# xdsopl/dwt

Measured on AMD Instinct MI355X. Metric: Mpixels/s lossless encode+decode round-trip, higher is better.
Workload: dtype int32; 1 GPU; 4096x4096x1 8-bit synthetic smooth+noise frames, lossless, 128 frames per GPU per step (BASELINE.json configs[1] geometry); frames_per_gpu=128, parallelism=1 GPU

## Files before the change

### dwt_amd/csrc/dwtx_internal.h

```cpp
#pragma once

#include <hip/hip_runtime.h>
#include <stdint.h>
#include <stddef.h>
#include "../../include/dwtx.h"

#define DWTX_SCRATCH_SLOTS 24
#define DWTX_PART_STREAMS 4
#define DWTX_ENC_PARTS DWTX_PART_STREAMS

struct dwtx_linplan;

struct dwtx_ctx {
	int device;
	hipStream_t stream;
	bool own_stream;
	void *scratch[DWTX_SCRATCH_SLOTS];
	size_t scratch_bytes[DWTX_SCRATCH_SLOTS];
	dwtx_linplan *plans;
	hipStream_t side[DWTX_PART_STREAMS - 1];
	int nside;
	struct { hipEvent_t start, cleared, tables[DWTX_PART_STREAMS], scattered[DWTX_PART_STREAMS]; } dec_ev;
	dwtx_ctx *enc_part[DWTX_ENC_PARTS];
	struct { hipEvent_t start, lifted[DWTX_ENC_PARTS], done[DWTX_ENC_PARTS]; } enc_ev;
// ... 180 lines not shown
	p.kind = DWTX_SAMPLE_U16;
	return p;
}
static inline dwtx_pixels dwtx_pixels_float(void *pix, int kind, int channels, size_t image_stride, int maxval)
{
	dwtx_pixels p{ pix, kind == DWTX_SAMPLE_F32 ? 4 : 2, channels, image_stride, maxval };
	p.kind = kind;
	return p;
}

bool dwtx_pixels_ok(const dwtx_pixels &px, int W, int H);
int dwtx_lift_scratch(dwtx_ctx *ctx, int W, int H, int nplanes);
int dwtx_pixels_to_planes(dwtx_ctx *ctx, int32_t *planes, const dwtx_pixels &px, int W, int H, int n);
int dwtx_planes_to_pixels(dwtx_ctx *ctx, const dwtx_pixels &px, const int32_t *planes, int W, int H, int n);

struct dwtx_tiles {
	int NT;
	int tile_first[DWTX_MAX_LEVELS + 1];
	const int *base;
	const unsigned short *cnt;
	const int *blk;
	const int *xy2tile;
	int xy_first[DWTX_MAX_LEVELS + 1];
	int nbs[DWTX_MAX_LEVELS];
};

struct dwtx_hist_sink {
	unsigned *cum32;
	unsigned *tile_mx;
	int NT, NTP;
	dwtx_tiles tiles;
};
int dwtx_hist_begin(dwtx_ctx *ctx, int W, int H, int C, int n, dwtx_hist_sink *sink);
struct dwtx_p16 {
	int16_t *planes;
	unsigned levels;
};
int dwtx_fwd_pixels(dwtx_ctx *ctx, int32_t *out, const dwtx_pixels &px, int W, int H, int n, const dwtx_hist_sink *sink = nullptr,
	unsigned *hist_levels = nullptr, dwtx_p16 p16 = dwtx_p16{ nullptr, 0u });
int dwtx_inv_pixels(dwtx_ctx *ctx, const dwtx_pixels &px, const int32_t *in, int W, int H, int n, const dwtx_p16 *p16 = nullptr);
int dwtx_transformation_fwd_hist(dwtx_ctx *ctx, int32_t *out, const int32_t *in, int W, int H, int nplanes, const dwtx_hist_sink *sink,
	unsigned *hist_levels);
int dwtx_get_tiles(dwtx_ctx *ctx, int W, int H, dwtx_tiles *out);

template <class G> int dwtx_fill_geom(dwtx_ctx *ctx, int W, int H, int C, G &g, dwtx_tiles &tiles)
{
	int lengths[DWTX_MAX_LEVELS], pixels[DWTX_MAX_LEVELS], widths[DWTX_MAX_LEVELS], heights[DWTX_MAX_LEVELS];
	g.levels = dwtx_compute_lengths(lengths, pixels, widths, heights, W, H, DWTX_MIN_LEN);
	for (int l = 0; l <= g.levels; ++l) {
		g.pixels[l] = pixels[l];
		g.side[l] = l < g.levels ? lengths[l + 1] : 0;
	}
	g.C = C;
	g.W = W;
	g.H = H;
	g.total = (long)W * H;
	g.pyr = nullptr;
	g.fine16 = nullptr;
	g.lv16 = 0u;
	g.sq_levels = 0;
	const int rc = dwtx_get_tiles(ctx, W, H, &tiles);
	if (rc)
		return rc;
	for (int l = 0; l <= g.levels; ++l)
		g.tile_first[l] = tiles.tile_first[l];
	g.tile_base = tiles.base;
	g.tile_cnt = tiles.cnt;
	g.tile_blk = tiles.blk;
	return DWTX_OK;
}

unsigned dwtx_square_levels(int W, int H);
unsigned dwtx_levels16(int W, int H, unsigned sq_levels);
int dwtx_linearization_ex(dwtx_ctx *ctx, int32_t *lin, const int32_t *pyr, int W, int H, int nplanes, unsigned skip_levels,
	dwtx_p16 p16 = dwtx_p16{ nullptr, 0u });
int dwtx_reconstruction_ex(dwtx_ctx *ctx, int32_t *pyr, const int32_t *lin, const int *dev_missing, int levels_out, int W, int H,
	int C, int n, unsigned skip_levels, dwtx_p16 p16 = dwtx_p16{ nullptr, 0u });
int dwtx_encode_planes_ex(dwtx_ctx *ctx, const int32_t *lin, const int32_t *pyr, unsigned sq_levels, unsigned hist_levels, int W, int H, int C, int n,
	long capacity, uint8_t *out, size_t out_stride, dwtx_stream_info *dev_info, dwtx_p16 p16 = dwtx_p16{ nullptr, 0u },
	dwtx_index *dev_index = nullptr);

constexpr unsigned DWTX_FUSED_FINE16 = 1u << 31;
int dwtx_decode_planes_ex(dwtx_ctx *ctx, int32_t *lin, int32_t *pyr, const uint8_t *streams, size_t stream_stride,
// ... 10 lines not shown
```

### dwt_amd/csrc/hilbert_dev.h

```cpp
#pragma once

#include "dwtx_internal.h"

namespace {

constexpr int BLK_LOG2 = 5;
constexpr int SQ_WORDS = 1024;

struct HilbertLow {
	unsigned short xy[1 << (2 * BLK_LOG2)];
};

constexpr HilbertLow make_hilbert_low()
{
	HilbertLow t{};
	for (unsigned i = 0; i < (1u << (2 * BLK_LOG2)); ++i) {
		unsigned x = 0, y = 0, d = i;
		for (unsigned s = 1; s < (1u << BLK_LOG2); s <<= 1) {
			const unsigned rx = (d >> 1) & 1u;
			const unsigned ry = (d ^ rx) & 1u;
			if (rx && !ry) {
				x ^= s - 1;
				y ^= s - 1;
			}
// ... 6 lines not shown
			y |= ry ? s : 0u;
			d >>= 2;
		}
		t.xy[i] = (unsigned short)(x | (y << 8));
	}
	return t;
}

__device__ const HilbertLow HILBERT_LOW = make_hilbert_low();

struct SquareMap {
	bool sw;
	unsigned mx, my;
};

__device__ __forceinline__ SquareMap square_map(int n, unsigned sq)
{
	SquareMap m = { false, 0u, 0u };
	for (unsigned s = 1u << BLK_LOG2; s < (unsigned)n; s <<= 1) {
		const unsigned rx = (sq >> 1) & 1u;
		const unsigned ry = (sq ^ rx) & 1u;
		if (rx && !ry) {
			m.mx ^= s - 1;
			m.my ^= s - 1;
		}
		if (!ry) {
			const unsigned t = m.mx;
			m.mx = m.my;
			m.my = t;
			m.sw = !m.sw;
		}
		m.mx ^= rx ? s : 0u;
		m.my ^= ry ? s : 0u;
		sq >>= 2;
	}
	return m;
}

__device__ __forceinline__ void hilbert_in_square(const SquareMap &m, int i, int &xo, int &yo)
{
	const unsigned e = HILBERT_LOW.xy[i];
	const unsigned xl = e & 255u, yl = e >> 8;
	xo = (int)((m.sw ? yl : xl) ^ m.mx);
	yo = (int)((m.sw ? xl : yl) ^ m.my);
}

__device__ __forceinline__ void sq_wave_sync()
{
	__builtin_amdgcn_fence(__ATOMIC_RELEASE, "wavefront");
	__builtin_amdgcn_wave_barrier();
	__builtin_amdgcn_fence(__ATOMIC_ACQUIRE, "wavefront");
}

// ... 19 lines not shown
{
	const unsigned a = m.mx & 31u, b = m.my & 31u;
	const unsigned key = (((b << 5) | (a ^ ((b & 7u) << 2))) << 2) * 0x00010001u;
	const unsigned short *tab = SQUARE_POS.off[m.sw ? 1 : 0];
	const uint4 e0 = *reinterpret_cast<const uint4 *>(tab + 16 * lane);
	const uint4 e1 = *reinterpret_cast<const uint4 *>(tab + 16 * lane + 8);
	const unsigned e[8] = { e0.x, e0.y, e0.z, e0.w, e1.x, e1.y, e1.z, e1.w };
#pragma unroll
	for (int k = 0; k < 8; ++k) {
		const unsigned w = e[k] ^ key;
		pos[2 * k] = w & 0xffffu;
		pos[2 * k + 1] = w >> 16;
	}
}

__device__ __forceinline__ void load_square16(const int *__restrict__ plane_pyr, int ppitch, int n, int blk, int lane,
	unsigned *lds, int (&val)[16])
{
	const SquareMap m = square_map(n, (unsigned)blk);
	const unsigned X0 = m.mx & ~31u, Y0 = m.my & ~31u;
#pragma unroll
	for (int it = 0; it < 4; ++it) {
		const int row = it * 8 + (lane >> 3), c4 = (lane & 7) * 4;
		const int4 v = *reinterpret_cast<const int4 *>(plane_pyr + (long)(Y0 + row) * ppitch + X0 + c4);
		*reinterpret_cast<int4 *>(lds + ((row << 5) | (c4 ^ ((row & 7) << 2)))) = v;
	}
	unsigned pos[16];
	square_positions16(m, lane, pos);
	sq_wave_sync();
	const char *base = reinterpret_cast<const char *>(lds);
#pragma unroll
	for (int k = 0; k < 16; ++k)
		val[k] = *reinterpret_cast<const int *>(base + pos[k]);
	sq_wave_sync();
}

__device__ __forceinline__ void store_square16(int *__restrict__ plane_pyr, int ppitch, int n, int blk, int lane, unsigned *lds,
	const int (&val)[16])
{
	const SquareMap m = square_map(n, (unsigned)blk);
	const unsigned X0 = m.mx & ~31u, Y0 = m.my & ~31u;
	unsigned pos[16];
	square_positions16(m, lane, pos);
	char *base = reinterpret_cast<char *>(lds);
#pragma unroll
	for (int k = 0; k < 16; ++k)
		*reinterpret_cast<int *>(base + pos[k]) = val[k];
	sq_wave_sync();
#pragma unroll
	for (int it = 0; it < 4; ++it) {
		const int row = it * 8 + (lane >> 3), c4 = (lane & 7) * 4;
		*reinterpret_cast<int4 *>(plane_pyr + (long)(Y0 + row) * ppitch + X0 + c4) =
			*reinterpret_cast<const int4 *>(lds + ((row << 5) | (c4 ^ ((row & 7) << 2))));
	}
	sq_wave_sync();
}

__device__ __forceinline__ void load_square16(const short *__restrict__ plane_pyr, int ppitch, int n, int blk, int lane,
	unsigned *lds, int (&val)[16])
{
	const SquareMap m = square_map(n, (unsigned)blk);
	const unsigned X0 = m.mx & ~31u, Y0 = m.my & ~31u;
#pragma unroll
	for (int it = 0; it < 2; ++it) {
		const int row = it * 16 + (lane >> 2), c8 = (lane & 3) * 8;
		const uint4 v = *reinterpret_cast<const uint4 *>(plane_pyr + (long)(Y0 + row) * ppitch + X0 + c8);
		const unsigned u[4] = { v.x, v.y, v.z, v.w };
#pragma unroll
		for (int h = 0; h < 2; ++h) {
			const int c4 = c8 + 4 * h;
			const int4 w = make_int4((int)(short)(u[2 * h] & 0xffffu), (int)u[2 * h] >> 16, (int)(short)(u[2 * h + 1] & 0xffffu), (int)u[2 * h + 1] >> 16);
			*reinterpret_cast<int4 *>(lds + ((row << 5) | (c4 ^ ((row & 7) << 2)))) = w;
		}
	}
	unsigned pos[16];
	square_positions16(m, lane, pos);
	sq_wave_sync();
	const char *base = reinterpret_cast<const char *>(lds);
#pragma unroll
	for (int k = 0; k < 16; ++k)
		val[k] = *reinterpret_cast<const int *>(base + pos[k]);
	sq_wave_sync();
}

__device__ __forceinline__ void store_square16(short *__restrict__ plane_pyr, int ppitch, int n, int blk, int lane, unsigned *lds,
	const int (&val)[16])
{
	const SquareMap m = square_map(n, (unsigned)blk);
	const unsigned X0 = m.mx & ~31u, Y0 = m.my & ~31u;
	unsigned pos[16];
	square_positions16(m, lane, pos);
	char *base = reinterpret_cast<char *>(lds);
#pragma unroll
	for (int k = 0; k < 16; ++k)
		*reinterpret_cast<int *>(base + pos[k]) = val[k];
	sq_wave_sync();
#pragma unroll
	for (int it = 0; it < 2; ++it) {
		const int row = it * 16 + (lane >> 2), c8 = (lane & 3) * 8;
		unsigned u[4];
#pragma unroll
		for (int h = 0; h < 2; ++h) {
			const int c4 = c8 + 4 * h;
// ... 12 lines not shown
```

### dwt_amd/csrc/linearize.hip

```cpp
#include "hilbert_dev.h"

#include <stdlib.h>
#include <string.h>
#include <new>
#include <vector>

namespace {

constexpr int THREADS = 256;

struct LinGeom {
	int levels;
	int W, H;
	int widths[DWTX_MAX_LEVELS], heights[DWTX_MAX_LEVELS], pixels[DWTX_MAX_LEVELS], lengths[DWTX_MAX_LEVELS];
	int blk_first[DWTX_MAX_LEVELS + 1];
	int blk_pts_log2[DWTX_MAX_LEVELS];
};

__device__ __forceinline__ void hilbert_d2xy(int n, unsigned d, int &xo, int &yo)
{
	unsigned x = 0, y = 0;
	for (unsigned s = 1; s < (unsigned)n; s <<= 1) {
		const unsigned rx = (d >> 1) & 1u;
		const unsigned ry = (d ^ rx) & 1u;
// ... 239 lines not shown

struct dwtx_linplan {
	int W, H;
	LinGeom g;
	int nblocks;
	int *d_blockbase;
	dwtx_tiles tiles;
	int *d_copy_list;
	int copy_upto[DWTX_MAX_LEVELS + 1];
	dwtx_linplan *next;
};

static void plan_destroy(dwtx_linplan *p)
{
	(void)hipFree(p->d_blockbase);
	(void)hipFree(const_cast<int *>(p->tiles.base));
	(void)hipFree(p->d_copy_list);
	(void)hipFree(const_cast<int *>(p->tiles.xy2tile));
	free(p);
}

static int build_plan(dwtx_ctx *ctx, dwtx_linplan *p, int W, int H)
{
	p->W = W;
	p->H = H;
	LinGeom &g = p->g;
	g.W = W;
	g.H = H;
	g.levels = dwtx_compute_lengths(g.lengths, g.pixels, g.widths, g.heights, W, H, DWTX_MIN_LEN);
	int nb = 0;
	for (int l = 0; l < g.levels; ++l) {
// ... 22 lines not shown
	std::vector<int> hb((size_t)(nb > 0 ? nb : 1));
	if (hipMemcpyAsync(hb.data(), p->d_blockbase, sizeof(int) * (size_t)nb, hipMemcpyDeviceToHost, ctx->stream) != hipSuccess ||
		hipStreamSynchronize(ctx->stream) != hipSuccess) {
		dwtx_set_error("plan download failed");
		return DWTX_ERR_DEVICE;
	}
	auto in_ring = [&](int l, int bb) {
		const int last = g.blk_first[l + 1], ring = g.pixels[l + 1] - g.pixels[l];
		return (bb + 1 < last ? hb[(size_t)bb + 1] : ring) - hb[(size_t)bb];
	};
	int nt = 0;
	for (int l = 0; l < g.levels; ++l)
		for (int bb = g.blk_first[l]; bb < g.blk_first[l + 1]; ++bb)
			nt += in_ring(l, bb) > 0;
	{
		const size_t o_blk = sizeof(int) * (size_t)nt, o_cnt = 2 * sizeof(int) * (size_t)nt;
		const size_t bytes = o_cnt + sizeof(unsigned short) * (size_t)nt + 64;
		std::vector<char> host(bytes);
		int *tb = (int *)host.data(), *tk = (int *)(host.data() + o_blk);
		unsigned short *tc = (unsigned short *)(host.data() + o_cnt);
		int t = 0;
		for (int l = 0; l < g.levels; ++l) {
			p->tiles.tile_first[l] = t;
			for (int bb = g.blk_first[l]; bb < g.blk_first[l + 1]; ++bb) {
				const int c = in_ring(l, bb);
				if (c <= 0)
					continue;
				tb[t] = hb[(size_t)bb];
				tk[t] = bb - g.blk_first[l];
				tc[t] = (unsigned short)c;
				++t;
			}
		}
		p->tiles.tile_first[g.levels] = t;
		p->tiles.NT = t;
		char *dev = nullptr;
		if (hipMalloc((void **)&dev, bytes) != hipSuccess) {
			dwtx_set_error("tile table hipMalloc failed");
			return DWTX_ERR_NOMEM;
		}
		p->tiles.base = (const int *)dev;
		p->tiles.blk = (const int *)(dev + o_blk);
		p->tiles.cnt = (const unsigned short *)(dev + o_cnt);
		if (hipMemcpy(dev, host.data(), bytes, hipMemcpyHostToDevice) != hipSuccess) {
			dwtx_set_error("tile table upload failed");
			return DWTX_ERR_DEVICE;
		}
	}
	{
		int total = 0;
		for (int l = 0; l < g.levels; ++l) {
			p->tiles.xy_first[l] = total;
			p->tiles.nbs[l] = g.lengths[l + 1] >= 64 ? g.lengths[l + 1] >> BLK_LOG2 : 0;
			total += p->tiles.nbs[l] * p->tiles.nbs[l];
		}
		p->tiles.xy_first[g.levels] = total;
		std::vector<int> tab((size_t)(total > 0 ? total : 1));
		for (int l = 0; l < g.levels; ++l) {
			const int nbs = p->tiles.nbs[l];
// ... 203 lines not shown
```

### dwt_amd/csrc/pack.hip

```cpp
#include "hilbert_dev.h"

#include <stdlib.h>
#include <string.h>

namespace {

constexpr int TILE = 1024;
constexpr int NCUM = 32;
constexpr int MAX_PLANES = 16;
constexpr int MAX_SEGS = 3 * 16 * MAX_PLANES;
constexpr int SUB = 64;
constexpr int CHUNK = SUB * 64;
constexpr int GROUP = 64;

constexpr unsigned T_RUN = 0x0fffu, T_ESC = 0x0fffu, T_BREAK = 1u << 13, T_VOID = 1u << 14, T_NOSIGN = 1u << 15;

struct PackGeom {
	int levels, C, W, H;
	long total;
	const int *pyr;
	const short *fine16;
	unsigned lv16;
	unsigned sq_levels;
	int side[DWTX_MAX_LEVELS + 1];
	int pixels[DWTX_MAX_LEVELS + 1];
	int tile_first[DWTX_MAX_LEVELS + 1];
	const int *tile_base;
	const unsigned short *tile_cnt;
	const int *tile_blk;
};

struct ImgInfo {
	int planes[3];
	int pmax;
	int K;
	int E;
	unsigned T;
	int order0;
	unsigned hdr_bits;
	unsigned root_bits;
	unsigned meta_bits;
	unsigned cut;
	unsigned long long total_bits;
	unsigned long long nbytes;
// ... 81 lines not shown
}
__device__ __forceinline__ int vli_top(int o, unsigned v) { return ilog2u(v + (1u << o)); }
__device__ __forceinline__ int vli_next(int top) { return top >= 2 ? top - 2 : 0; }

__device__ __forceinline__ void seg_unpack(int d, int &c, int &l, int &p)
{
	c = d & 15;
	l = (d >> 4) & 15;
	p = (d >> 8) - 1;
}

struct __attribute__((packed, aligned(4))) Int4U {
	int x, y, z, w;
};

__device__ __forceinline__ void load_tile16(const PackGeom &g, const int *__restrict__ lin, int plane, int l, int tile, int lane, int nvalid,
	int nv, unsigned *lds, int (&val)[16])
{
	if (((g.sq_levels >> l) & 1u) && nvalid == TILE) {
		if ((g.lv16 >> l) & 1u)
			load_square16(g.fine16 + (long)plane * g.total, g.W, g.side[l], g.tile_blk[tile], lane, lds, val);
		else
			load_square16(g.pyr + (long)plane * g.total, g.W, g.side[l], g.tile_blk[tile], lane, lds, val);
		return;
	}
	const int tbase = g.tile_base[tile];
	const int *src = lin + (long)plane * g.total + g.pixels[l] + tbase + 16 * lane;
	const int k = (int)(((uintptr_t)src >> 2) & 3);
	const bool last_of_ring = g.pixels[l] + (long)tbase + TILE >= g.pixels[l + 1];
	if (nvalid == TILE && (k == 0 || !last_of_ring)) {
		const int4 *A = reinterpret_cast<const int4 *>(src - k);
		int t[20];
#pragma unroll
		for (int q = 0; q < 4; ++q) {
			const int4 v4 = A[q];
			t[4 * q] = v4.x;
			t[4 * q + 1] = v4.y;
			t[4 * q + 2] = v4.z;
			t[4 * q + 3] = v4.w;
		}
		t[16] = t[17] = t[18] = t[19] = 0;
		if (k) {
			const int4 v4 = A[4];
			t[16] = v4.x;
// ... 21 lines not shown
			for (int i = 0; i < 16; ++i)
				val[i] = t[i + 3];
			break;
		}
	} else {
#pragma unroll
		for (int i = 0; i < 16; ++i)
			val[i] = i < nv ? src[i] : 0;
	}
}


__device__ __forceinline__ void hist_load(const PackGeom &g, const int *__restrict__ lin, int plane, int tile, int lane, int (&val)[16],
	unsigned &ok, int &nvalid)
{
	int l = 0;
	while (l + 1 < g.levels && tile >= g.tile_first[l + 1])
		++l;
	const long base = g.pixels[l] + g.tile_base[tile];
	nvalid = g.tile_cnt[tile];
	ok = 0xffffu;
	if (((g.sq_levels >> l) & 1u) && nvalid == TILE) {
		const SquareMap m = square_map(g.side[l], (unsigned)g.tile_blk[tile]);
		const long at = (long)plane * g.total + (long)(m.my & ~31u) * g.W + (m.mx & ~31u);
		if ((g.lv16 >> l) & 1u) {
			const short *sq = g.fine16 + at;
#pragma unroll
			for (int it = 0; it < 2; ++it) {
				const uint4 v4 = *reinterpret_cast<const uint4 *>(sq + (long)(it * 16 + (lane >> 2)) * g.W + (lane & 3) * 8);
				const unsigned u[4] = { v4.x, v4.y, v4.z, v4.w };
#pragma unroll
				for (int k = 0; k < 4; ++k) {
					val[8 * it + 2 * k] = (int)(short)(u[k] & 0xffffu);
					val[8 * it + 2 * k + 1] = (int)u[k] >> 16;
				}
			}
		} else {
			const int *sq = g.pyr + at;
// ... 79 lines not shown
		cum[lane] = (unsigned short)(lane == NCUM - 1 ? (mx ? ilog2u(mx) + 1 : 0) : nvalid);
	}
	if (lane == 0)
		w.tile_mx[(long)plane * w.NTP + tile] = mx;
}

constexpr int HIST_TPW = 2;

__global__ __launch_bounds__(256) void k_hist_init(PackGeom g, Work w)
{
	const int i = blockIdx.x * blockDim.x + threadIdx.x;
	const int plane = blockIdx.y;
	if (i >= w.NT * (NCUM / 2))
		return;
	const int tile = i / (NCUM / 2), d = i - tile * (NCUM / 2);
	const unsigned cnt = g.tile_cnt[tile];
	reinterpret_cast<unsigned *>(w.cum + ((long)plane * w.NT + tile) * NCUM)[d] = d < 8 ? 0u : d < 15 ? cnt * 0x00010001u : cnt;
	if (d == 0)
		w.tile_mx[(long)plane * w.NTP + tile] = 0u;
}

__global__ __launch_bounds__(256) void k_hist(PackGeom g, const int *__restrict__ lin, Work w, unsigned done_levels)
{
	const int lane = threadIdx.x & 63;
	const int tile0 = (blockIdx.x * 4 + wave_in_block()) * HIST_TPW;
	const int plane = blockIdx.y;
	if (tile0 >= w.NT)
		return;
	if (done_levels) {
		int l = 0;
		while (l + 1 < g.levels && tile0 >= g.tile_first[l + 1])
			++l;
		const bool d0 = (done_levels >> l) & 1u;
		const bool same = tile0 + 1 < g.tile_first[l + 1];
		const bool d1 = same ? d0 : (l + 1 < g.levels ? ((done_levels >> (l + 1)) & 1u) != 0 : true);
		if (d0 && d1)
			return;
		if (d0 != d1) {
			const int t = d0 ? tile0 + 1 : tile0;
			if (t < w.NT) {
				int val1[16], nv1;
				unsigned ok1;
				hist_load(g, lin, plane, t, lane, val1, ok1, nv1);
				hist_finish(w, plane, t, lane, val1, ok1, nv1);
			}
			return;
		}
// ... 715 lines not shown
		for (int p = P > 0 ? P - 1 : 0; p >= 0; --p) {
			const int ones = (int)(cum_s(p + 1) - cum_s(p));
			const unsigned gb = ent_s(p) >= 0 ? (unsigned)__builtin_amdgcn_readlane((int)my_tokbase, p) : ~0u;
			if (ones <= 0 || gb == ~0u)
				continue;
			plane_out(gb, (unsigned)__builtin_amdgcn_readlane((int)my_slot0, p), ones);
		}
	}

#undef ZL
#undef CT
}

template <bool WIDE>
__device__ __forceinline__ void code_one(const PackGeom &g, const int *__restrict__ lin, const Work &w, CodeLds &L, const unsigned char *pext4, int tile,
	int plane, int lane)
{
	const int img = plane / g.C, c = plane - img * g.C;
	const ImgInfo &I = w.info[img];
	{
	int l = 0;
	while (l + 1 < g.levels && tile >= g.tile_first[l + 1])
		++l;
	const int j = tile - g.tile_first[l];
	const int nvalid = g.tile_cnt[tile];
	const int P = I.planes[c] < MAX_PLANES ? I.planes[c] : MAX_PLANES;
	const unsigned live = w.live[(long)img * 48 + c * 16 + l];
	if (!live)
		return;
	const unsigned tile_or = w.tile_mx[(long)plane * w.NTP + tile];
	const int tile_top = tile_or ? ilog2u(tile_or) + 1 : 0;
	if (!(live & ((1u << (tile_top < 31 ? tile_top : 31)) - 1u))) {
		if (lane < MAX_PLANES && ((live >> lane) & 1u)) {
			const int k = w.segidx[((long)img * 48 + c * 16 + l) * MAX_PLANES + lane] - 1;
			w.ent_tz[img * w.ES + w.seg_ebase[(long)img * (MAX_SEGS + 1) + k] + j] = (unsigned short)nvalid;
		}
		return;
	}
	const int first = 16 * lane;
	const int nv = nvalid - first < 0 ? 0 : nvalid - first > 16 ? 16 : nvalid - first;
	const int vb = first < nvalid ? first : nvalid;

	static_assert(sizeof(L.tab) >= sizeof(unsigned) * SQ_WORDS, "the class table doubles as the square's staging area");
	int val[16];
	load_tile16(g, lin, plane, l, tile, lane, nvalid, nv, L.tab, val);
	unsigned my_tokbase = 0;
	int my_ent = -1;
	unsigned long long my_rb = 0;
	if (lane < MAX_PLANES) {
		const int p = lane;
		const int k1 = (live >> p) & 1u ? w.segidx[((long)img * 48 + c * 16 + l) * MAX_PLANES + p] : 0;
		if (k1) {
			const int k = k1 - 1;
			const int e0 = w.seg_ebase[(long)img * (MAX_SEGS + 1) + k];
			my_ent = e0 + j;
			my_rb = (unsigned long long)w.ent_refw[img * (w.ES + 1) + my_ent] << 5;
			my_tokbase = w.ent_tokbase[img * (w.ES + 1) + my_ent];
		}
	}
	if (!WIDE) {
		if (nvalid == TILE)
			code_tile<8, true>(L, pext4, val, w, img, lane, nvalid, nv, vb, P, tile_top, my_tokbase, my_ent, my_rb);
		else
			code_tile<8, false>(L, pext4, val, w, img, lane, nvalid, nv, vb, P, tile_top, my_tokbase, my_ent, my_rb);
	} else {
		code_tile<16, false>(L, pext4, val, w, img, lane, nvalid, nv, vb, P, tile_top, my_tokbase, my_ent, my_rb);
	}
	}
}

template <bool WIDE>
__global__ __launch_bounds__(256) __attribute__((amdgpu_waves_per_eu(5))) void k_code(PackGeom g, const int *__restrict__ lin, Work w)
{
	__shared__ CodeLds lds[4];
	__shared__ unsigned char pext4[256];
	const int lane = threadIdx.x & 63, wv = WIDE ? (int)(threadIdx.x >> 6) : wave_in_block();
	const int plane = blockIdx.y;
	const int img = plane / g.C, c = plane - img * g.C;
	if ((w.info[img].planes[c] > 8) != WIDE)
		return;
	if (!WIDE) {
		pext4[threadIdx.x] = (unsigned char)pext4_entry(threadIdx.x);
		__syncthreads();
		const int tile = blockIdx.x * 4 + wv;
		if (tile < w.NT)
			code_one<false>(g, lin, w, lds[wv], pext4, tile, plane, lane);
	} else {
		for (int tile = blockIdx.x * 4 + wv; tile < w.NT; tile += gridDim.x * 4) {
			code_one<true>(g, lin, w, lds[wv], pext4, tile, plane, lane);
			wave_sync();
		}
	}
}


__device__ __forceinline__ RunMap compose(RunMap a, RunMap b)
{
	RunMap r;
	r.keep = a.keep & b.keep;
	r.add = b.keep ? a.add + b.add : b.add;
	return r;
}

__device__ __forceinline__ void token_store(const Work &w, int img, unsigned t, unsigned run, unsigned flags)
// ... 1107 lines not shown
}


extern "C" int dwtx_encode_planes(dwtx_ctx *ctx, const int32_t *lin, int W, int H, int C, int n, long capacity,
	uint8_t *out, size_t out_stride, dwtx_stream_info *dev_info)
{
	return dwtx_encode_planes_ex(ctx, lin, nullptr, 0u, 0u, W, H, C, n, capacity, out, out_stride, dev_info, dwtx_p16{ nullptr, 0u },
		ctx ? ctx->enc_index : nullptr);
}

static int pack_geometry(dwtx_ctx *ctx, int W, int H, int C, int n, PackGeom &g, Work &w, dwtx_tiles &tiles)
{
	const int rc = dwtx_fill_geom(ctx, W, H, C, g, tiles);
	if (rc)
		return rc;
	memset(&w, 0, sizeof(w));
	w.NT = tiles.NT;
	w.NTP = (tiles.NT + 3) / 4 * 4;
	const size_t nplanes = (size_t)n * C;
	const bool ok = carve(ctx, SLOT_PK_CUM, [&](Carve &c) {
		c.take(w.cum, nplanes * w.NT * NCUM);
		c.take(w.tile_mx, nplanes * w.NTP);
	});
	return ok ? DWTX_OK : DWTX_ERR_NOMEM;
}

int dwtx_hist_begin(dwtx_ctx *ctx, int W, int H, int C, int n, dwtx_hist_sink *sink)
{
	if (!ctx || !sink || (C != 1 && C != 3) || n < 1 || !dwtx_count_ok((long)n * C, DWTX_MAX_PLANES_PER_CALL, "planes"))
		return DWTX_ERR_ARG;
// ... 129 lines not shown
	if (!w.sublut || !ch)
		return DWTX_ERR_NOMEM;

	hipStream_t s = ctx->stream;
	const long out_words = (long)(out_stride / 4);
	unsigned *outw = (unsigned *)out;

	if (hist_tiles > 0)
		hipLaunchKernelGGL(k_hist, dim3(dwtx_cdiv(hist_tiles, 4 * HIST_TPW), nplanes), dim3(256), 0, s, g, lin, w, hist_levels);
	hipLaunchKernelGGL(k_plan, dim3(n), dim3(1024), 0, s, g, lin, w, outw, out_words, capacity);
	hipLaunchKernelGGL(k_entries_count, dim3((unsigned)w.NCB, n), dim3(ENT_BLOCK), 0, s, g, w);
	hipLaunchKernelGGL(k_entries_blocks, dim3(n), dim3(ENT_BLOCK), 0, s, w);
	hipLaunchKernelGGL(k_entries_finish, dim3((unsigned)w.NCB, n), dim3(ENT_BLOCK), 0, s, w);
	hipLaunchKernelGGL(k_entries_segs, dim3(n), dim3(ENT_BLOCK), 0, s, w);
	hipLaunchKernelGGL(k_cut, dim3(n), dim3(ENT_BLOCK), 0, s, w, capacity, (int)(ctx->opt[DWTX_OPT_NO_CAPACITY_CUT] != 0));
	hipLaunchKernelGGL(k_code<false>, dim3(dwtx_cdiv(NT, 4), nplanes), dim3(256), 0, s, g, lin, w);
	hipLaunchKernelGGL(k_code<true>, dim3(dwtx_cdiv(NT, 4) < 64 ? dwtx_cdiv(NT, 4) : 64, nplanes), dim3(256), 0, s, g, lin, w);
	hipLaunchKernelGGL(k_carry_local, dim3((unsigned)w.NCB, n), dim3(CARRY_THREADS), 0, s, w);
	hipLaunchKernelGGL(k_carry_blocks, dim3(n), dim3(CARRY_BLOCK), 0, s, w);
	if (dev_index)
		hipLaunchKernelGGL(k_carry_apply<true>, dim3((unsigned)w.NCB, n), dim3(CARRY_THREADS), 0, s, w);
	else
		hipLaunchKernelGGL(k_carry_apply<false>, dim3((unsigned)w.NCB, n), dim3(CARRY_THREADS), 0, s, w);
	hipLaunchKernelGGL(k_gorder, dim3((int)((w.NCS + GO_WAVES - 1) / GO_WAVES), n), dim3(64 * GO_WAVES), 0, s, w);
	hipLaunchKernelGGL(k_lut, dim3(512, n), dim3(256), 0, s, w);
	hipLaunchKernelGGL(k_chain_groups, dim3(64, n), dim3(256), 0, s, w);
	hipLaunchKernelGGL(k_chain_image, dim3(n), dim3(1024), 0, s, w);
	hipLaunchKernelGGL(k_gorder_exact, dim3(512, n), dim3(256), 0, s, w);
	hipLaunchKernelGGL(k_bitscan, dim3(n), dim3(1024), 0, s, w, capacity);
	{
		const long cb = (out_words / 4 + 256) / 256;
		hipLaunchKernelGGL(k_clear_stream, dim3((unsigned)(cb < 1024 ? cb : 1024), n), dim3(256), 0, s, w, outw, out_words);
// ... 11 lines not shown
```

### dwt_amd/csrc/unpack.hip

```cpp
#include "hilbert_dev.h"

#include <stdlib.h>
#include <string.h>
#include <vector>

namespace {

constexpr int TILE = 1024;
constexpr int MAX_PLANES = 16;
constexpr int MAX_SEGS = 3 * 16 * MAX_PLANES;
constexpr int CH_LOG2 = 7;
constexpr int CH_BITS = 1 << CH_LOG2;
constexpr int SCAN_BLOCK = 1024;
constexpr int LINK_ROUNDS = 12;
constexpr int FAM = 2;

struct UnpackGeom {
	int levels, C, W, H;
	long total;
	long lin_stride;
	int pixels[DWTX_MAX_LEVELS + 1];
	int tile_first[DWTX_MAX_LEVELS + 1];
	int levels_max;
	int *pyr;
	short *fine16;
	unsigned lv16;
	unsigned sq_levels;
	int side[DWTX_MAX_LEVELS + 1];
	const int *tile_base;
	const unsigned short *tile_cnt;
	const int *tile_blk;
};

struct DecInfo {
	int status;
	int W, H, C;
	int levels;
	int planes[3];
	int pmax;
	int level;
	int nsegs;
	int truncated;
	int missing[48];
	unsigned long long bits_used;
	unsigned hops, hopped_chunks;
	unsigned walked_tokens;
// ... 1666 lines not shown
			rank[i] = cy + woff + inc - v;
		__syncthreads();
		if (threadIdx.x == 0)
			carry = cy + all;
		__syncthreads();
	}
}

__global__ __launch_bounds__(256) void k_count(UnpackGeom g, DWork w, int p)
{
	const int tile = blockIdx.x * blockDim.x + threadIdx.x;
	const int plane = blockIdx.y;
	const int img = plane / g.C;
	if (tile >= w.NT)
		return;
	int l = 0;
	while (l + 1 < g.levels && tile >= g.tile_first[l + 1])
		++l;
	const unsigned long long cb = w.count_base[(long)plane * 16 + l];
	if (!cb)
		return;
	unsigned short *ns = w.tile_nonsig + (long)plane * w.NT + tile;
	unsigned *rk = w.tile_rank + ((long)plane * MAX_PLANES + p) * w.NT + tile;
	const unsigned n = *ns;
	if (!n)
		return;
	const unsigned *sym = w.symbits + img * w.BW;
	const unsigned long long a = cb - 1ull + 2ull * *rk;
	const unsigned long long e = a + 2ull * n;
	const long first = (long)(a >> 5), last = (long)((e - 1) >> 5);
	unsigned ones = 0;
#pragma unroll 4
	for (long w0 = first & ~3l; w0 <= last; w0 += 4) {
// ... 71 lines not shown

struct __attribute__((packed, aligned(4))) Int4S {
	int x, y, z, w;
};

__global__ __launch_bounds__(256) __attribute__((amdgpu_waves_per_eu(6))) void k_apply_all(UnpackGeom g, DWork w, const unsigned char *streams, long stream_stride, int *lin)
{
	__shared__ __attribute__((aligned(16))) unsigned char dep[sizeof(DepositTables)];
	static_assert(sizeof(DepositTables) == 17 * 256, "one 16-byte piece and one byte per thread");
	*reinterpret_cast<uint4 *>(dep + 16 * threadIdx.x) = *reinterpret_cast<const uint4 *>(DEPOSIT.sym + 16 * threadIdx.x);
	dep[4096 + threadIdx.x] = DEPOSIT.ref[threadIdx.x];
	__syncthreads();
	const unsigned char *dsym = dep, *dref = dep + 4096;
	const int lane = threadIdx.x & 63, wv = wave_in_block();
	const int tile = blockIdx.x * 4 + wv;
	const int plane = blockIdx.y;
	if (tile >= w.NT)
		return;
	const int img = plane / g.C, c = plane - img * g.C;
	const DecInfo &I = w.info[img];
	if (I.status)
		return;
	int l = 0;
	while (l + 1 < g.levels && tile >= g.tile_first[l + 1])
		++l;
	const unsigned tbase = (unsigned)g.tile_base[tile];
	const long base = g.pixels[l] + (long)tbase;
	const int nvalid = g.tile_cnt[tile];
	const int first = 16 * lane;
	const int nv = nvalid - first < 0 ? 0 : nvalid - first > 16 ? 16 : nvalid - first;
	const int vb = first < nvalid ? first : nvalid;
	const unsigned *sym = w.symbits + img * w.BW;
	const unsigned *stream = (const unsigned *)(streams + img * stream_stride);
	const long stream_words = stream_stride >> 2;
	unsigned R[8] = { 0u, 0u, 0u, 0u, 0u, 0u, 0u, 0u };
	int p_last = 0, rows_in = 0;
	auto push_row = [&](unsigned row16) {
		if (rows_in >= 8) {
#pragma unroll
			for (int k = 7; k >= 4; --k)
				R[k] = __builtin_amdgcn_alignbit(R[k], R[k - 1], 16);
		}
		if (rows_in >= 6)
// ... 141 lines not shown
		for (int i = 0; i < 16; ++i)
			mag[i] <<= p_last;
	}
	if (((g.sq_levels >> l) & 1u) && nvalid == TILE) {
		const int m = I.missing[c * 16 + l] - 2;
		const int bias = m >= 0 ? 1 << m : 0;
		int val[16];
#pragma unroll
		for (int i = 0; i < 16; ++i) {
			int v = ((neg >> i) & 1u) ? -(int)mag[i] : (int)mag[i];
			if (bias && v)
				v += v < 0 ? -bias : bias;
			val[i] = v;
		}
		if ((g.lv16 >> l) & 1u)
			store_square16(g.fine16 + (long)plane * g.lin_stride, g.W, g.side[l], g.tile_blk[tile], lane, ap_mem[wv], val);
		else
			store_square16(g.pyr + (long)plane * g.lin_stride, g.W, g.side[l], g.tile_blk[tile], lane, ap_mem[wv], val);
		return;
	}
	int *dst = lin + (long)plane * g.lin_stride + base + first;
	if (nvalid == TILE) {
#pragma unroll
		for (int q = 0; q < 4; ++q) {
			Int4S v;
			v.x = ((neg >> (4 * q)) & 1u) ? -(int)mag[4 * q] : (int)mag[4 * q];
			v.y = ((neg >> (4 * q + 1)) & 1u) ? -(int)mag[4 * q + 1] : (int)mag[4 * q + 1];
			v.z = ((neg >> (4 * q + 2)) & 1u) ? -(int)mag[4 * q + 2] : (int)mag[4 * q + 2];
			v.w = ((neg >> (4 * q + 3)) & 1u) ? -(int)mag[4 * q + 3] : (int)mag[4 * q + 3];
			*reinterpret_cast<Int4S *>(dst + 4 * q) = v;
		}
	} else {
#pragma unroll
		for (int i = 0; i < 16; ++i)
			if (i < nv)
				dst[i] = ((neg >> i) & 1u) ? -(int)mag[i] : (int)mag[i];
	}
}

__global__ __launch_bounds__(256) void k_tiles_init(UnpackGeom g, DWork w, int nplanes)
{
	const int tile = blockIdx.x * blockDim.x + threadIdx.x;
	const int plane = blockIdx.y;
	if (tile >= w.NT || plane >= nplanes)
		return;
	int l = 0;
	while (l + 1 < g.levels && tile >= g.tile_first[l + 1])
		++l;
	w.tile_nonsig[(long)plane * w.NT + tile] = g.tile_cnt[tile];
}

__global__ __launch_bounds__(256) void k_nch(DWork w, const unsigned long long *lens, int n)
{
	const int i = blockIdx.x * blockDim.x + threadIdx.x;
	if (i >= n)
		return;
	const unsigned long long bits = lens[i] * 8ull;
	long c = (long)((bits + CH_BITS - 1) / CH_BITS);
	c = (c + 1 + 3) / 4 * 4 - 1;
	w.nch[i] = (int)(c < w.NCH ? c : w.NCH);
}

}

// ... 287 lines not shown
		const bool every_plane = ctx->opt[DWTX_OPT_COUNT_EVERY_PLANE] != 0;
		for (int b = pmax - 1; b >= 0; --b) {
			hipLaunchKernelGGL(k_rank, dim3(g.levels, p.count * C), dim3(1024), 0, p.stream, g, h, b, every_plane);
			hipLaunchKernelGGL(k_count, dim3(dwtx_cdiv(w.NT, 256), p.count * C), dim3(256), 0, p.stream, g, h, b);
		}
		bool whole = sq_all != 0;
		for (int i = p.first; i < end; ++i)
			whole = whole && !host_info[i].status && host_info[i].level == g.levels - 1;
		UnpackGeom ga = g;
		ga.sq_levels = whole ? sq_all : 0u;
		ga.pyr = whole ? pyr + (size_t)p.first * C * g.lin_stride : nullptr;
		const bool fine = whole && p16.planes && p16.levels && !((uintptr_t)p16.planes & 15) && !(p16.levels & ~sq_all) && pmax <= 15;
		ga.fine16 = fine ? p16.planes + (size_t)p.first * C * g.lin_stride : nullptr;
		ga.lv16 = fine ? p16.levels : 0u;
		p.fused = ga.sq_levels | (fine ? DWTX_FUSED_FINE16 : 0u);
		hipLaunchKernelGGL(k_apply_all, dim3(dwtx_cdiv(w.NT, 4), p.count * C), dim3(256), 0, p.stream, ga, h,
			streams + (size_t)p.first * stream_stride, (long)stream_stride, lin + (size_t)p.first * C * g.lin_stride);
		DWTX_LAUNCH_CHECK();
		return DWTX_OK;
	}

	int run(DecPart *part, int K, int (*done)(void *user, int first, int count, unsigned fused_levels), void *user)
	{
		int rc;
		for (int k = 0; k < K; ++k) {
			DecPart &p = part[k];
			if (k > 0)
				DWTX_HIP(hipStreamWaitEvent(p.stream, ctx->dec_ev.tables[k - 1], 0));
			if ((rc = chunk_tables(p.stream, p.first, p.count, fam0)))
				return rc;
			if (k + 1 < K)
// ... 79 lines not shown
```

Before: 94070 Mpixels/s.

## Pack per-tile metadata into one 16-byte record with precomputed square map

Replaces the separate tile base, count and block arrays with a packed 16-byte record per tile. The record holds base, absolute offset, count, level and the precomputed Hilbert square map, built on the host. Device kernels now load this record in one access instead of scanning tile_first in a loop to find the level and recomputing square_map per tile. The coding and apply kernels also move image and channel onto separate grid dimensions, which removes an integer division. The cost is a larger table in memory and the limits the packing imposes, which are checked with static asserts.

```diff
diff --git a/dwt_amd/csrc/dwtx_internal.h b/dwt_amd/csrc/dwtx_internal.h
--- a/dwt_amd/csrc/dwtx_internal.h
+++ b/dwt_amd/csrc/dwtx_internal.h
@@ -218,12 +218,19 @@
 int dwtx_pixels_to_planes(dwtx_ctx *ctx, int32_t *planes, const dwtx_pixels &px, int W, int H, int n);
 int dwtx_planes_to_pixels(dwtx_ctx *ctx, const dwtx_pixels &px, const int32_t *planes, int W, int H, int n);
 
+struct dwtx_tile_rec {
+	int base, at;
+	unsigned info, masks;
+};
+static_assert(sizeof(dwtx_tile_rec) == 16, "a tile's record is one 16-byte load");
+constexpr int DWTX_REC_LEVEL_SHIFT = 16, DWTX_REC_SWAP_SHIFT = 31;
+static_assert(DWTX_MAX_SIDE <= (1 << 15), "a square map's XOR mask is below the curve's side: 16 bits each hold it");
+static_assert(DWTX_MAX_LEVELS <= 16, "the record keeps the level in four bits");
 struct dwtx_tiles {
 	int NT;
 	int tile_first[DWTX_MAX_LEVELS + 1];
-	const int *base;
+	const dwtx_tile_rec *rec;
 	const unsigned short *cnt;
-	const int *blk;
 	const int *xy2tile;
 	int xy_first[DWTX_MAX_LEVELS + 1];
 	int nbs[DWTX_MAX_LEVELS];
@@ -251,10 +258,8 @@
 {
 	int lengths[DWTX_MAX_LEVELS], pixels[DWTX_MAX_LEVELS], widths[DWTX_MAX_LEVELS], heights[DWTX_MAX_LEVELS];
 	g.levels = dwtx_compute_lengths(lengths, pixels, widths, heights, W, H, DWTX_MIN_LEN);
-	for (int l = 0; l <= g.levels; ++l) {
+	for (int l = 0; l <= g.levels; ++l)
 		g.pixels[l] = pixels[l];
-		g.side[l] = l < g.levels ? lengths[l + 1] : 0;
-	}
 	g.C = C;
 	g.W = W;
 	g.H = H;
@@ -268,9 +273,7 @@
 		return rc;
 	for (int l = 0; l <= g.levels; ++l)
 		g.tile_first[l] = tiles.tile_first[l];
-	g.tile_base = tiles.base;
-	g.tile_cnt = tiles.cnt;
-	g.tile_blk = tiles.blk;
+	g.tile_rec = tiles.rec;
 	return DWTX_OK;
 }
 
diff --git a/dwt_amd/csrc/hilbert_dev.h b/dwt_amd/csrc/hilbert_dev.h
--- a/dwt_amd/csrc/hilbert_dev.h
+++ b/dwt_amd/csrc/hilbert_dev.h
@@ -44,7 +44,7 @@
 	unsigned mx, my;
 };
 
-__device__ __forceinline__ SquareMap square_map(int n, unsigned sq)
+__host__ __device__ __forceinline__ SquareMap square_map(int n, unsigned sq)
 {
 	SquareMap m = { false, 0u, 0u };
 	for (unsigned s = 1u << BLK_LOG2; s < (unsigned)n; s <<= 1) {
@@ -67,6 +67,37 @@
 	return m;
 }
 
+struct TileRec {
+	int base;
+	int at;
+	int cnt, l;
+	SquareMap map;
+};
+
+__host__ __device__ __forceinline__ dwtx_tile_rec tile_rec_pack(int base, int at, int cnt, int l, const SquareMap &m)
+{
+	dwtx_tile_rec r;
+	r.base = base;
+	r.at = at;
+	r.info = (unsigned)cnt | (unsigned)l << DWTX_REC_LEVEL_SHIFT | (m.sw ? 1u : 0u) << DWTX_REC_SWAP_SHIFT;
+	r.masks = m.mx | m.my << 16;
+	return r;
+}
+
+__device__ __forceinline__ TileRec tile_rec(const dwtx_tile_rec *__restrict__ recs, int tile)
+{
+	const uint4 r = reinterpret_cast<const uint4 *>(recs)[tile];
+	TileRec t;
+	t.base = (int)r.x;
+	t.at = (int)r.y;
+	t.cnt = (int)(r.z & 0xffffu);
+	t.l = (int)((r.z >> DWTX_REC_LEVEL_SHIFT) & 15u);
+	t.map.sw = (r.z >> DWTX_REC_SWAP_SHIFT) != 0u;
+	t.map.mx = r.w & 0xffffu;
+	t.map.my = r.w >> 16;
+	return t;
+}
+
 __device__ __forceinline__ void hilbert_in_square(const SquareMap &m, int i, int &xo, int &yo)
 {
 	const unsigned e = HILBERT_LOW.xy[i];
@@ -116,10 +147,9 @@
 	}
 }
 
-__device__ __forceinline__ void load_square16(const int *__restrict__ plane_pyr, int ppitch, int n, int blk, int lane,
+__device__ __forceinline__ void load_square16(const int *__restrict__ plane_pyr, int ppitch, const SquareMap &m, int lane,
 	unsigned *lds, int (&val)[16])
 {
-	const SquareMap m = square_map(n, (unsigned)blk);
 	const unsigned X0 = m.mx & ~31u, Y0 = m.my & ~31u;
 #pragma unroll
 	for (int it = 0; it < 4; ++it) {
@@ -137,10 +167,9 @@
 	sq_wave_sync();
 }
 
-__device__ __forceinline__ void store_square16(int *__restrict__ plane_pyr, int ppitch, int n, int blk, int lane, unsigned *lds,
+__device__ __forceinline__ void store_square16(int *__restrict__ plane_pyr, int ppitch, const SquareMap &m, int lane, unsigned *lds,
 	const int (&val)[16])
 {
-	const SquareMap m = square_map(n, (unsigned)blk);
 	const unsigned X0 = m.mx & ~31u, Y0 = m.my & ~31u;
 	unsigned pos[16];
 	square_positions16(m, lane, pos);
@@ -158,10 +187,9 @@
 	sq_wave_sync();
 }
 
-__device__ __forceinline__ void load_square16(const short *__restrict__ plane_pyr, int ppitch, int n, int blk, int lane,
+__device__ __forceinline__ void load_square16(const short *__restrict__ plane_pyr, int ppitch, const SquareMap &m, int lane,
 	unsigned *lds, int (&val)[16])
 {
-	const SquareMap m = square_map(n, (unsigned)blk);
 	const unsigned X0 = m.mx & ~31u, Y0 = m.my & ~31u;
 #pragma unroll
 	for (int it = 0; it < 2; ++it) {
@@ -185,10 +213,9 @@
 	sq_wave_sync();
 }
 
-__device__ __forceinline__ void store_square16(short *__restrict__ plane_pyr, int ppitch, int n, int blk, int lane, unsigned *lds,
+__device__ __forceinline__ void store_square16(short *__restrict__ plane_pyr, int ppitch, const SquareMap &m, int lane, unsigned *lds,
 	const int (&val)[16])
 {
-	const SquareMap m = square_map(n, (unsigned)blk);
 	const unsigned X0 = m.mx & ~31u, Y0 = m.my & ~31u;
 	unsigned pos[16];
 	square_positions16(m, lane, pos);
diff --git a/dwt_amd/csrc/linearize.hip b/dwt_amd/csrc/linearize.hip
--- a/dwt_amd/csrc/linearize.hip
+++ b/dwt_amd/csrc/linearize.hip
@@ -277,7 +277,7 @@
 static void plan_destroy(dwtx_linplan *p)
 {
 	(void)hipFree(p->d_blockbase);
-	(void)hipFree(const_cast<int *>(p->tiles.base));
+	(void)hipFree(const_cast<dwtx_tile_rec *>(p->tiles.rec));
 	(void)hipFree(p->d_copy_list);
 	(void)hipFree(const_cast<int *>(p->tiles.xy2tile));
 	free(p);
@@ -330,11 +330,7 @@
 		for (int bb = g.blk_first[l]; bb < g.blk_first[l + 1]; ++bb)
 			nt += in_ring(l, bb) > 0;
 	{
-		const size_t o_blk = sizeof(int) * (size_t)nt, o_cnt = 2 * sizeof(int) * (size_t)nt;
-		const size_t bytes = o_cnt + sizeof(unsigned short) * (size_t)nt + 64;
-		std::vector<char> host(bytes);
-		int *tb = (int *)host.data(), *tk = (int *)(host.data() + o_blk);
-		unsigned short *tc = (unsigned short *)(host.data() + o_cnt);
+		std::vector<dwtx_tile_rec> host((size_t)(nt > 0 ? nt : 1));
 		int t = 0;
 		for (int l = 0; l < g.levels; ++l) {
 			p->tiles.tile_first[l] = t;
@@ -342,23 +338,25 @@
 				const int c = in_ring(l, bb);
 				if (c <= 0)
 					continue;
-				tb[t] = hb[(size_t)bb];
-				tk[t] = bb - g.blk_first[l];
-				tc[t] = (unsigned short)c;
-				++t;
+				const int base = hb[(size_t)bb];
+				host[(size_t)t++] = tile_rec_pack(base, g.pixels[l] + base, c, l, square_map(g.lengths[l + 1], (unsigned)(bb - g.blk_first[l])));
 			}
 		}
 		p->tiles.tile_first[g.levels] = t;
 		p->tiles.NT = t;
+		const size_t rec_bytes = sizeof(dwtx_tile_rec) * host.size();
+		std::vector<unsigned short> cnt(host.size());
+		for (int i = 0; i < t; ++i)
+			cnt[(size_t)i] = (unsigned short)(host[(size_t)i].info & 0xffffu);
 		char *dev = nullptr;
-		if (hipMalloc((void **)&dev, bytes) != hipSuccess) {
+		if (hipMalloc((void **)&dev, rec_bytes + sizeof(unsigned short) * cnt.size()) != hipSuccess) {
 			dwtx_set_error("tile table hipMalloc failed");
 			return DWTX_ERR_NOMEM;
 		}
-		p->tiles.base = (const int *)dev;
-		p->tiles.blk = (const int *)(dev + o_blk);
-		p->tiles.cnt = (const unsigned short *)(dev + o_cnt);
-		if (hipMemcpy(dev, host.data(), bytes, hipMemcpyHostToDevice) != hipSuccess) {
+		p->tiles.rec = (const dwtx_tile_rec *)dev;
+		p->tiles.cnt = (const unsigned short *)(dev + rec_bytes);
+		if (hipMemcpy(dev, host.data(), rec_bytes, hipMemcpyHostToDevice) != hipSuccess ||
+			hipMemcpy(dev + rec_bytes, cnt.data(), sizeof(unsigned short) * cnt.size(), hipMemcpyHostToDevice) != hipSuccess) {
 			dwtx_set_error("tile table upload failed");
 			return DWTX_ERR_DEVICE;
 		}
diff --git a/dwt_amd/csrc/pack.hip b/dwt_amd/csrc/pack.hip
--- a/dwt_amd/csrc/pack.hip
+++ b/dwt_amd/csrc/pack.hip
@@ -22,12 +22,10 @@
 	const short *fine16;
 	unsigned lv16;
 	unsigned sq_levels;
-	int side[DWTX_MAX_LEVELS + 1];
 	int pixels[DWTX_MAX_LEVELS + 1];
 	int tile_first[DWTX_MAX_LEVELS + 1];
-	const int *tile_base;
+	const dwtx_tile_rec *tile_rec;
 	const unsigned short *tile_cnt;
-	const int *tile_blk;
 };
 
 struct ImgInfo {
@@ -139,20 +137,20 @@
 	int x, y, z, w;
 };
 
-__device__ __forceinline__ void load_tile16(const PackGeom &g, const int *__restrict__ lin, int plane, int l, int tile, int lane, int nvalid,
+__device__ __forceinline__ void load_tile16(const PackGeom &g, const int *__restrict__ lin, int plane, const TileRec &tr, int lane,
 	int nv, unsigned *lds, int (&val)[16])
 {
+	const int l = tr.l, nvalid = tr.cnt;
 	if (((g.sq_levels >> l) & 1u) && nvalid == TILE) {
 		if ((g.lv16 >> l) & 1u)
-			load_square16(g.fine16 + (long)plane * g.total, g.W, g.side[l], g.tile_blk[tile], lane, lds, val);
+			load_square16(g.fine16 + (long)plane * g.total, g.W, tr.map, lane, lds, val);
 		else
-			load_square16(g.pyr + (long)plane * g.total, g.W, g.side[l], g.tile_blk[tile], lane, lds, val);
+			load_square16(g.pyr + (long)plane * g.total, g.W, tr.map, lane, lds, val);
 		return;
 	}
-	const int tbase = g.tile_base[tile];
-	const int *src = lin + (long)plane * g.total + g.pixels[l] + tbase + 16 * lane;
+	const int *src = lin + (long)plane * g.total + tr.at + 16 * lane;
 	const int k = (int)(((uintptr_t)src >> 2) & 3);
-	const bool last_of_ring = g.pixels[l] + (long)tbase + TILE >= g.pixels[l + 1];
+	const bool last_of_ring = (long)tr.at + TILE >= g.pixels[l + 1];
 	if (nvalid == TILE && (k == 0 || !last_of_ring)) {
 		const int4 *A = reinterpret_cast<const int4 *>(src - k);
 		int t[20];
@@ -204,14 +202,13 @@
 __device__ __forceinline__ void hist_load(const PackGeom &g, const int *__restrict__ lin, int plane, int tile, int lane, int (&val)[16],
 	unsigned &ok, int &nvalid)
 {
-	int l = 0;
-	while (l + 1 < g.levels && tile >= g.tile_first[l + 1])
-		++l;
-	const long base = g.pixels[l] + g.tile_base[tile];
-	nvalid = g.tile_cnt[tile];
+	const TileRec tr = tile_rec(g.tile_rec, tile);
+	const int l = tr.l;
+	const long base = tr.at;
+	nvalid = tr.cnt;
 	ok = 0xffffu;
 	if (((g.sq_levels >> l) & 1u) && nvalid == TILE) {
-		const SquareMap m = square_map(g.side[l], (unsigned)g.tile_blk[tile]);
+		const SquareMap &m = tr.map;
 		const long at = (long)plane * g.total + (long)(m.my & ~31u) * g.W + (m.mx & ~31u);
 		if ((g.lv16 >> l) & 1u) {
 			const short *sq = g.fine16 + at;
@@ -321,7 +318,7 @@
 	if (i >= w.NT * (NCUM / 2))
 		return;
 	const int tile = i / (NCUM / 2), d = i - tile * (NCUM / 2);
-	const unsigned cnt = g.tile_cnt[tile];
+	const unsigned cnt = (unsigned)tile_rec(g.tile_rec, tile).cnt;
 	reinterpret_cast<unsigned *>(w.cum + ((long)plane * w.NT + tile) * NCUM)[d] = d < 8 ? 0u : d < 15 ? cnt * 0x00010001u : cnt;
 	if (d == 0)
 		w.tile_mx[(long)plane * w.NTP + tile] = 0u;
@@ -335,9 +332,7 @@
 	if (tile0 >= w.NT)
 		return;
 	if (done_levels) {
-		int l = 0;
-		while (l + 1 < g.levels && tile0 >= g.tile_first[l + 1])
-			++l;
+		const int l = tile_rec(g.tile_rec, tile0).l;
 		const bool d0 = (done_levels >> l) & 1u;
 		const bool same = tile0 + 1 < g.tile_first[l + 1];
 		const bool d1 = same ? d0 : (l + 1 < g.levels ? ((done_levels >> (l + 1)) & 1u) != 0 : true);
@@ -1083,16 +1078,15 @@
 
 template <bool WIDE>
 __device__ __forceinline__ void code_one(const PackGeom &g, const int *__restrict__ lin, const Work &w, CodeLds &L, const unsigned char *pext4, int tile,
-	int plane, int lane)
-{
-	const int img = plane / g.C, c = plane - img * g.C;
+	int img, int c, int lane)
+{
+	const int plane = img * g.C + c;
 	const ImgInfo &I = w.info[img];
 	{
-	int l = 0;
-	while (l + 1 < g.levels && tile >= g.tile_first[l + 1])
-		++l;
+	const TileRec tr = tile_rec(g.tile_rec, tile);
+	const int l = tr.l;
 	const int j = tile - g.tile_first[l];
-	const int nvalid = g.tile_cnt[tile];
+	const int nvalid = tr.cnt;
 	const int P = I.planes[c] < MAX_PLANES ? I.planes[c] : MAX_PLANES;
 	const unsigned live = w.live[(long)img * 48 + c * 16 + l];
 	if (!live)
@@ -1112,7 +1106,7 @@
 
 	static_assert(sizeof(L.tab) >= sizeof(unsigned) * SQ_WORDS, "the class table doubles as the square's staging area");
 	int val[16];
-	load_tile16(g, lin, plane, l, tile, lane, nvalid, nv, L.tab, val);
+	load_tile16(g, lin, plane, tr, lane, nv, L.tab, val);
 	unsigned my_tokbase = 0;
 	int my_ent = -1;
 	unsigned long long my_rb = 0;
@@ -1143,9 +1137,8 @@
 {
 	__shared__ CodeLds lds[4];
 	__shared__ unsigned char pext4[256];
-	const int lane = threadIdx.x & 63, wv = WIDE ? (int)(threadIdx.x >> 6) : wave_in_block();
-	const int plane = blockIdx.y;
-	const int img = plane / g.C, c = plane - img * g.C;
+	const int lane = threadIdx.x & 63, wv = wave_in_block();
+	const int c = blockIdx.y, img = blockIdx.z;
 	if ((w.info[img].planes[c] > 8) != WIDE)
 		return;
 	if (!WIDE) {
@@ -1153,10 +1146,10 @@
 		__syncthreads();
 		const int tile = blockIdx.x * 4 + wv;
 		if (tile < w.NT)
-			code_one<false>(g, lin, w, lds[wv], pext4, tile, plane, lane);
+			code_one<false>(g, lin, w, lds[wv], pext4, tile, img, c, lane);
 	} else {
 		for (int tile = blockIdx.x * 4 + wv; tile < w.NT; tile += gridDim.x * 4) {
-			code_one<true>(g, lin, w, lds[wv], pext4, tile, plane, lane);
+			code_one<true>(g, lin, w, lds[wv], pext4, tile, img, c, lane);
 			wave_sync();
 		}
 	}
@@ -2294,6 +2287,7 @@
 	const int rc = dwtx_fill_geom(ctx, W, H, C, g, tiles);
 	if (rc)
 		return rc;
+	g.tile_cnt = tiles.cnt;
 	memset(&w, 0, sizeof(w));
 	w.NT = tiles.NT;
 	w.NTP = (tiles.NT + 3) / 4 * 4;
@@ -2453,8 +2447,8 @@
 	hipLaunchKernelGGL(k_entries_finish, dim3((unsigned)w.NCB, n), dim3(ENT_BLOCK), 0, s, w);
 	hipLaunchKernelGGL(k_entries_segs, dim3(n), dim3(ENT_BLOCK), 0, s, w);
 	hipLaunchKernelGGL(k_cut, dim3(n), dim3(ENT_BLOCK), 0, s, w, capacity, (int)(ctx->opt[DWTX_OPT_NO_CAPACITY_CUT] != 0));
-	hipLaunchKernelGGL(k_code<false>, dim3(dwtx_cdiv(NT, 4), nplanes), dim3(256), 0, s, g, lin, w);
-	hipLaunchKernelGGL(k_code<true>, dim3(dwtx_cdiv(NT, 4) < 64 ? dwtx_cdiv(NT, 4) : 64, nplanes), dim3(256), 0, s, g, lin, w);
+	hipLaunchKernelGGL(k_code<false>, dim3(dwtx_cdiv(NT, 4), C, n), dim3(256), 0, s, g, lin, w);
+	hipLaunchKernelGGL(k_code<true>, dim3(dwtx_cdiv(NT, 4) < 64 ? dwtx_cdiv(NT, 4) : 64, C, n), dim3(256), 0, s, g, lin, w);
 	hipLaunchKernelGGL(k_carry_local, dim3((unsigned)w.NCB, n), dim3(CARRY_THREADS), 0, s, w);
 	hipLaunchKernelGGL(k_carry_blocks, dim3(n), dim3(CARRY_BLOCK), 0, s, w);
 	if (dev_index)
diff --git a/dwt_amd/csrc/unpack.hip b/dwt_amd/csrc/unpack.hip
--- a/dwt_amd/csrc/unpack.hip
+++ b/dwt_amd/csrc/unpack.hip
@@ -26,10 +26,7 @@
 	short *fine16;
 	unsigned lv16;
 	unsigned sq_levels;
-	int side[DWTX_MAX_LEVELS + 1];
-	const int *tile_base;
-	const unsigned short *tile_cnt;
-	const int *tile_blk;
+	const dwtx_tile_rec *tile_rec;
 };
 
 struct DecInfo {
@@ -1726,9 +1723,7 @@
 	const int img = plane / g.C;
 	if (tile >= w.NT)
 		return;
-	int l = 0;
-	while (l + 1 < g.levels && tile >= g.tile_first[l + 1])
-		++l;
+	const int l = tile_rec(g.tile_rec, tile).l;
 	const unsigned long long cb = w.count_base[(long)plane * 16 + l];
 	if (!cb)
 		return;
@@ -1830,19 +1825,18 @@
 	const unsigned char *dsym = dep, *dref = dep + 4096;
 	const int lane = threadIdx.x & 63, wv = wave_in_block();
 	const int tile = blockIdx.x * 4 + wv;
-	const int plane = blockIdx.y;
+	const int c = blockIdx.y, img = blockIdx.z;
+	const int plane = img * g.C + c;
 	if (tile >= w.NT)
 		return;
-	const int img = plane / g.C, c = plane - img * g.C;
 	const DecInfo &I = w.info[img];
 	if (I.status)
 		return;
-	int l = 0;
-	while (l + 1 < g.levels && tile >= g.tile_first[l + 1])
-		++l;
-	const unsigned tbase = (unsigned)g.tile_base[tile];
-	const long base = g.pixels[l] + (long)tbase;
-	const int nvalid = g.tile_cnt[tile];
+	const TileRec tr = tile_rec(g.tile_rec, tile);
+	const int l = tr.l;
+	const unsigned tbase = (unsigned)tr.base;
+	const long base = tr.at;
+	const int nvalid = tr.cnt;
 	const int first = 16 * lane;
 	const int nv = nvalid - first < 0 ? 0 : nvalid - first > 16 ? 16 : nvalid - first;
 	const int vb = first < nvalid ? first : nvalid;
@@ -2014,9 +2008,9 @@
 			val[i] = v;
 		}
 		if ((g.lv16 >> l) & 1u)
-			store_square16(g.fine16 + (long)plane * g.lin_stride, g.W, g.side[l], g.tile_blk[tile], lane, ap_mem[wv], val);
+			store_square16(g.fine16 + (long)plane * g.lin_stride, g.W, tr.map, lane, ap_mem[wv], val);
 		else
-			store_square16(g.pyr + (long)plane * g.lin_stride, g.W, g.side[l], g.tile_blk[tile], lane, ap_mem[wv], val);
+			store_square16(g.pyr + (long)plane * g.lin_stride, g.W, tr.map, lane, ap_mem[wv], val);
 		return;
 	}
 	int *dst = lin + (long)plane * g.lin_stride + base + first;
@@ -2044,10 +2038,7 @@
 	const int plane = blockIdx.y;
 	if (tile >= w.NT || plane >= nplanes)
 		return;
-	int l = 0;
-	while (l + 1 < g.levels && tile >= g.tile_first[l + 1])
-		++l;
-	w.tile_nonsig[(long)plane * w.NT + tile] = g.tile_cnt[tile];
+	w.tile_nonsig[(long)plane * w.NT + tile] = (unsigned short)tile_rec(g.tile_rec, tile).cnt;
 }
 
 __global__ __launch_bounds__(256) void k_nch(DWork w, const unsigned long long *lens, int n)
@@ -2365,7 +2356,7 @@
 		ga.fine16 = fine ? p16.planes + (size_t)p.first * C * g.lin_stride : nullptr;
 		ga.lv16 = fine ? p16.levels : 0u;
 		p.fused = ga.sq_levels | (fine ? DWTX_FUSED_FINE16 : 0u);
-		hipLaunchKernelGGL(k_apply_all, dim3(dwtx_cdiv(w.NT, 4), p.count * C), dim3(256), 0, p.stream, ga, h,
+		hipLaunchKernelGGL(k_apply_all, dim3(dwtx_cdiv(w.NT, 4), C, p.count), dim3(256), 0, p.stream, ga, h,
 			streams + (size_t)p.first * stream_stride, (long)stream_stride, lin + (size_t)p.first * C * g.lin_stride);
 		DWTX_LAUNCH_CHECK();
 		return DWTX_OK;
```

New measurement: 98480 Mpixels/s (median of 6 runs). 4.7% higher.
